# tdunnlab/scrubvae

Measured on AMD Instinct MI355X. Metric: pose-windows/sec (ELBO-match) on synthetic 64-frame mouse skeletons, higher is better.
Workload: dtype f32 (f16x3b3 split on the fp16 / bf16 matrix cores); 1 GPU; configs[2] full SC-VAE (conditional + grad_reversal x2 + adversarial_net), AdamW, batch 4096/GPU, window 64, 23 joints, z=32, channels [64,128,256,512,1024]; batch_per_gpu=4096, global_batch=4096, window=64, joints=23, launch=eager launches, inputs=resident in HBM, side_streams=2, parallelism=dp1, backend=none, ranks_seen=1, bn=single rank

## Files before the change

### scrubvae_amd/csrc/pose_tail.hip

```cpp
#include "svae_internal.h"
#include <cstdlib>

namespace svae {

struct TailArgs {
  const float* y;
  const float* offsets;
  const float* target;
  const float* root;
  const float* ext_dx6d;
  const float* ext_droot;
  float* x6d_hat;
  float* root_hat;
  float* loss_part;
  float* dy;
  float* pose_out;
  long long rows;
  int ld, J, ldt, ldo;
  int has_arena;
  int pre_tanh;
  float a0[3], a1[3];
  float jpe_scale, root_scale;
  svae_tree tree;
};

struct M3 {
  float m[9];
};

__device__ __forceinline__ M3 mul(const M3& a, const M3& b) {
  M3 c;
#pragma unroll
  for (int r = 0; r < 3; ++r)
#pragma unroll
    for (int k = 0; k < 3; ++k) c.m[r * 3 + k] = a.m[r * 3] * b.m[k] + a.m[r * 3 + 1] * b.m[3 + k] + a.m[r * 3 + 2] * b.m[6 + k];
  return c;
}
__device__ __forceinline__ M3 mul_tn(const M3& a, const M3& b) {
  M3 c;
#pragma unroll
  for (int r = 0; r < 3; ++r)
#pragma unroll
    for (int k = 0; k < 3; ++k) c.m[r * 3 + k] = a.m[r] * b.m[k] + a.m[3 + r] * b.m[3 + k] + a.m[6 + r] * b.m[6 + k];
  return c;
}
__device__ __forceinline__ M3 mul_nt(const M3& a, const M3& b) {
  M3 c;
#pragma unroll
  for (int r = 0; r < 3; ++r)
#pragma unroll
    for (int k = 0; k < 3; ++k)
      c.m[r * 3 + k] = a.m[r * 3] * b.m[k * 3] + a.m[r * 3 + 1] * b.m[k * 3 + 1] + a.m[r * 3 + 2] * b.m[k * 3 + 2];
  return c;
}

__device__ __forceinline__ void cross3(const float* a, const float* b, float* c) {
  c[0] = a[1] * b[2] - a[2] * b[1];
  c[1] = a[2] * b[0] - a[0] * b[2];
  c[2] = a[0] * b[1] - a[1] * b[0];
}

constexpr float K1_EPS = 1e-8f;

__device__ __forceinline__ M3 c6_to_mat(const float* a) {
  const float nx = sqrtf(a[0] * a[0] + a[1] * a[1] + a[2] * a[2]);
  const float ix = 1.f / (nx + K1_EPS);
  const float x[3] = {a[0] * ix, a[1] * ix, a[2] * ix};
  float zr[3];
  cross3(x, a + 3, zr);
  const float nz = sqrtf(zr[0] * zr[0] + zr[1] * zr[1] + zr[2] * zr[2]);
  const float iz = 1.f / (nz + K1_EPS);
  const float z[3] = {zr[0] * iz, zr[1] * iz, zr[2] * iz};
  float yv[3];
  cross3(z, x, yv);
  M3 M;
#pragma unroll
  for (int r = 0; r < 3; ++r) { M.m[r * 3] = x[r]; M.m[r * 3 + 1] = yv[r]; M.m[r * 3 + 2] = z[r]; }
  return M;
}

__device__ __forceinline__ void c6_to_mat_bwd(const float* a, const M3& dM, float* da) {
  const float nx = sqrtf(a[0] * a[0] + a[1] * a[1] + a[2] * a[2]);
  const float ix = 1.f / (nx + K1_EPS);
  const float x[3] = {a[0] * ix, a[1] * ix, a[2] * ix};
  float zr[3];
  cross3(x, a + 3, zr);
  const float nz = sqrtf(zr[0] * zr[0] + zr[1] * zr[1] + zr[2] * zr[2]);
  const float iz = 1.f / (nz + K1_EPS);
  const float z[3] = {zr[0] * iz, zr[1] * iz, zr[2] * iz};
  float gx[3] = {dM.m[0], dM.m[3], dM.m[6]}, gy[3] = {dM.m[1], dM.m[4], dM.m[7]}, gz[3] = {dM.m[2], dM.m[5], dM.m[8]};
  float t[3];
  cross3(x, gy, t);
  gz[0] += t[0]; gz[1] += t[1]; gz[2] += t[2];
  cross3(gy, z, t);
  gx[0] += t[0]; gx[1] += t[1]; gx[2] += t[2];
  const float dzr_dot = zr[0] * gz[0] + zr[1] * gz[1] + zr[2] * gz[2];
  const float kz = nz > 0.f ? dzr_dot * iz * iz / nz : 0.f;
  const float gzr[3] = {gz[0] * iz - zr[0] * kz, gz[1] * iz - zr[1] * kz, gz[2] * iz - zr[2] * kz};
  cross3(a + 3, gzr, t);
  gx[0] += t[0]; gx[1] += t[1]; gx[2] += t[2];
  cross3(gzr, x, da + 3);
  const float dx_dot = a[0] * gx[0] + a[1] * gx[1] + a[2] * gx[2];
  const float kx = nx > 0.f ? dx_dot * ix * ix / nx : 0.f;
  da[0] = gx[0] * ix - a[0] * kx;
  da[1] = gx[1] * ix - a[1] * kx;
  da[2] = gx[2] * ix - a[2] * kx;
}

template <int TR>
__global__ __launch_bounds__(64 * SVAE_MAX_CHAINS) void pose_tail_kernel(const TailArgs g) {
  extern __shared__ __attribute__((aligned(16))) float smem[];
  const int tid = threadIdx.x, nth = blockDim.x;
  const int wave = tid >> 6, lane = tid & 63;
  const int J = g.J, J3 = 3 * J, C6 = 6 * J;
  const int ldt = g.ldt, ldo = g.ldo;
  float* tile = smem;
  float* offs = tile + TR * ldt;
  float* pose = offs + TR * ldo;
  float* dm0 = pose + TR * ldo;
  float* red = dm0 + TR * 9;
  const long long r0 = (long long)blockIdx.x * TR;
  const int nrows = (int)((g.rows - r0) < TR ? (g.rows - r0) : TR);
  const int n_chains = g.tree.n_chains;

  {
    const int f4_per_row = g.ld / 4;
    const int total = nrows * f4_per_row;
    const float* src = g.y + r0 * g.ld;
    for (int e = tid; e < total; e += nth) {
      const int rr = e / f4_per_row, c = (e - rr * f4_per_row) * 4;
      const float4 v = *reinterpret_cast<const float4*>(src + (long long)e * 4);
      float* d = tile + rr * ldt + c;
      if (g.pre_tanh) { d[0] = tanhf(v.x); d[1] = tanhf(v.y); d[2] = tanhf(v.z); d[3] = tanhf(v.w); }
      else { d[0] = v.x; d[1] = v.y; d[2] = v.z; d[3] = v.w; }
    }
    const int tot3 = nrows * J3;
    const float* so = g.offsets + r0 * J3;
    for (int e = tid; e < tot3; e += nth) {
      const int rr = e / J3, c = e - rr * J3;
      offs[rr * ldo + c] = so[e];
    }
    for (int e = tid; e < TR * 9; e += nth) dm0[e] = 0.f;
  }
  __syncthreads();
  {
    const int tot6 = nrows * C6;
    float* dst = g.x6d_hat + r0 * C6;
    for (int e = tid; e < tot6; e += nth) {
      const int rr = e / C6, c = e - rr * C6;
      dst[e] = tile[rr * ldt + c];
    }
    if (g.has_arena) {
      float* dr = g.root_hat + r0 * 3;
      for (int e = tid; e < nrows * 3; e += nth) {
        const int rr = e / 3, k = e - rr * 3;
        dr[e] = 0.5f * (tile[rr * ldt + C6 + k] + 1.f) * (g.a1[k] - g.a0[k]) + g.a0[k];
      }
    }
  }

  const bool active = lane < nrows;
  const int lrow = lane < TR ? lane : 0;
  float* my = tile + lrow * ldt;
  float* myo = offs + lrow * ldo;
  float* myp = pose + lrow * ldo;
  const bool do_bwd = g.dy != nullptr;
  const bool chain_wave = wave < n_chains && g.tree.chain_len[wave < n_chains ? wave : 0] >= 2;
  const int ch = wave < n_chains ? wave : 0;
  const int len = g.tree.chain_len[ch];

  float a6[6];
  M3 M0;
  if (active) {
#pragma unroll
    for (int k = 0; k < 6; ++k) a6[k] = my[k];
    M0 = c6_to_mat(a6);
  }
  M3 Rc = M0;
  if (active && chain_wave) {
    M3& R = Rc;
    float acc[3] = {0.f, 0.f, 0.f};
    for (int i = 1; i < len; ++i) {
      const int j = g.tree.chain[ch][i];
#pragma unroll
      for (int k = 0; k < 6; ++k) a6[k] = my[6 * j + k];
      R = mul(R, c6_to_mat(a6));
      const float o0 = myo[3 * j], o1 = myo[3 * j + 1], o2 = myo[3 * j + 2];
#pragma unroll
      for (int r = 0; r < 3; ++r) {
        acc[r] += R.m[r * 3] * o0 + R.m[r * 3 + 1] * o1 + R.m[r * 3 + 2] * o2;
        myp[3 * j + r] = acc[r];
      }
    }
  }
  __syncthreads();

  float rl = 0.f;
  if (wave == 0 && active) {
    myp[0] = 0.f; myp[1] = 0.f; myp[2] = 0.f;
    for (int c = 0; c < n_chains; ++c) {
      const int cl = g.tree.chain_len[c];
      const int head = g.tree.chain[c][0];
      const float h0 = myp[3 * head], h1 = myp[3 * head + 1], h2 = myp[3 * head + 2];
      for (int i = 1; i < cl; ++i) {
        const int j = g.tree.chain[c][i];
        myp[3 * j] += h0; myp[3 * j + 1] += h1; myp[3 * j + 2] += h2;
      }
    }
  }
  const int root_wave = nth > 64 ? 1 : 0;
  if (wave == root_wave && active && g.has_arena) {
#pragma unroll
    for (int k = 0; k < 3; ++k) {
      const float xh = my[C6 + k];
      const float half = 0.5f * (g.a1[k] - g.a0[k]);
      const float rh = (xh + 1.f) * half + g.a0[k];
      const float d = rh - g.root[(r0 + lane) * 3 + k];
      rl += d * d;
      if (do_bwd) {
        float gk = 2.f * g.root_scale * d;
        if (g.ext_droot) gk += g.ext_droot[(r0 + lane) * 3 + k];
        my[C6 + k] = g.pre_tanh ? gk * half * (1.f - xh * xh) : gk * half;
      }
    }
  }
  if (wave == root_wave && active && do_bwd) {
    for (int c = C6 + (g.has_arena ? 3 : 0); c < g.ld; ++c) my[c] = 0.f;
  }
  __syncthreads();

  {
    float jpe = 0.f;
    const int tot3 = nrows * J3;
    const float* stg = g.target + r0 * J3;
    float* dp = g.pose_out ? g.pose_out + r0 * J3 : nullptr;
    for (int e = tid; e < tot3; e += nth) {
      const int rr = e / J3, c = e - rr * J3;
      const float pv = pose[rr * ldo + c];
      if (dp) dp[e] = pv;
      const float d = pv - stg[e];
      jpe += d * d;
      pose[rr * ldo + c] = 2.f * g.jpe_scale * d;
    }
    jpe = wave_sum(jpe);
    if (lane == 0) red[wave] = jpe;
  }
  __syncthreads();
  if (tid == 0) {
    float t = 0.f;
    for (int w = 0; w < nth / 64; ++w) t += red[w];
    g.loss_part[blockIdx.x * 2] = t;
  }
  if (do_bwd && wave == 0 && active) {
    for (int c = n_chains - 1; c >= 0; --c) {
      const int cl = g.tree.chain_len[c];
      for (int i = cl - 1; i >= 1; --i) {
        const int j = g.tree.chain[c][i], par = g.tree.chain[c][i - 1];
#pragma unroll
        for (int r = 0; r < 3; ++r) myp[3 * par + r] += myp[3 * j + r];
      }
    }
  }
  if (do_bwd) __syncthreads();

  M3 carry;
#pragma unroll
  for (int k = 0; k < 9; ++k) carry.m[k] = 0.f;
  if (do_bwd && active && chain_wave) {
    M3 P = Rc;
#pragma unroll
    for (int i = SVAE_MAX_CHAIN_LEN - 1; i >= 1; --i) {
      if (i < len) {
        const int j = g.tree.chain[ch][i];
        M3 D = carry;
#pragma unroll
        for (int r = 0; r < 3; ++r)
#pragma unroll
          for (int k = 0; k < 3; ++k) D.m[r * 3 + k] += myp[3 * j + r] * myo[3 * j + k];
#pragma unroll
        for (int k = 0; k < 6; ++k) a6[k] = my[6 * j + k];
        const M3 Mj = c6_to_mat(a6);
        {
          float inv[3];
#pragma unroll
          for (int c = 0; c < 3; ++c) inv[c] = 1.f / (Mj.m[c] * Mj.m[c] + Mj.m[3 + c] * Mj.m[3 + c] + Mj.m[6 + c] * Mj.m[6 + c]);
          M3 Q;
#pragma unroll
          for (int r = 0; r < 3; ++r)
#pragma unroll
            for (int k = 0; k < 3; ++k)
              Q.m[r * 3 + k] = P.m[r * 3] * inv[0] * Mj.m[k * 3] + P.m[r * 3 + 1] * inv[1] * Mj.m[k * 3 + 1] + P.m[r * 3 + 2] * inv[2] * Mj.m[k * 3 + 2];
          P = Q;
        }
        const M3 dMj = mul_tn(P, D);
        carry = mul_nt(D, Mj);
        float da[6];
        c6_to_mat_bwd(a6, dMj, da);
#pragma unroll
        for (int k = 0; k < 6; ++k) {
          float gk = da[k];
          if (g.ext_dx6d) gk += g.ext_dx6d[(r0 + lane) * C6 + 6 * j + k];
          my[6 * j + k] = g.pre_tanh ? gk * (1.f - a6[k] * a6[k]) : gk;
        }
      }
    }
  }
  if (do_bwd) {
    for (int c = 0; c < n_chains; ++c) {
      if (wave == c && chain_wave && active) {
        float* d = dm0 + lane * 9;
#pragma unroll
        for (int k = 0; k < 9; ++k) d[k] += carry.m[k];
      }
      __syncthreads();
    }
  }
  if (do_bwd && wave == 0 && active) {
    M3 dM0;
    const float* d = dm0 + lane * 9;
#pragma unroll
    for (int k = 0; k < 9; ++k) dM0.m[k] = d[k];
    float a0[6], da0[6];
#pragma unroll
    for (int k = 0; k < 6; ++k) a0[k] = my[k];
    c6_to_mat_bwd(a0, dM0, da0);
#pragma unroll
    for (int k = 0; k < 6; ++k) {
      float gk = da0[k];
      if (g.ext_dx6d) gk += g.ext_dx6d[(r0 + lane) * C6 + k];
      my[k] = g.pre_tanh ? gk * (1.f - a0[k] * a0[k]) : gk;
    }
  }
  if (wave == root_wave) {
    rl = wave_sum(rl);
    if (lane == 0) g.loss_part[blockIdx.x * 2 + 1] = rl;
  }
  __syncthreads();
  if (do_bwd) {
    const int f4_per_row = g.ld / 4;
    const int total = nrows * f4_per_row;
    float* dst = g.dy + r0 * g.ld;
    for (int e = tid; e < total; e += nth) {
      const int rr = e / f4_per_row, c = (e - rr * f4_per_row) * 4;
      const float* sp = tile + rr * ldt + c;
      *reinterpret_cast<float4*>(dst + (long long)e * 4) = make_float4(sp[0], sp[1], sp[2], sp[3]);
    }
  }
}

__device__ __forceinline__ void rot6d_rows(const float* d6, float* m ) {
  const float n1 = fmaxf(sqrtf(d6[0] * d6[0] + d6[1] * d6[1] + d6[2] * d6[2]), 1e-12f);
  const float b1[3] = {d6[0] / n1, d6[1] / n1, d6[2] / n1};
  const float dt = b1[0] * d6[3] + b1[1] * d6[4] + b1[2] * d6[5];
  const float u[3] = {d6[3] - dt * b1[0], d6[4] - dt * b1[1], d6[5] - dt * b1[2]};
  const float n2 = fmaxf(sqrtf(u[0] * u[0] + u[1] * u[1] + u[2] * u[2]), 1e-12f);
  const float b2[3] = {u[0] / n2, u[1] / n2, u[2] / n2};
  float b3[3];
  cross3(b1, b2, b3);
#pragma unroll
  for (int k = 0; k < 3; ++k) { m[k] = b1[k]; m[3 + k] = b2[k]; m[6 + k] = b3[k]; }
}

__device__ __forceinline__ void rot6d_rows_bwd(const float* d6, const float* g, float* dd) {
  const float n1r = sqrtf(d6[0] * d6[0] + d6[1] * d6[1] + d6[2] * d6[2]);
  const float n1 = fmaxf(n1r, 1e-12f);
  const float b1[3] = {d6[0] / n1, d6[1] / n1, d6[2] / n1};
  const float dt = b1[0] * d6[3] + b1[1] * d6[4] + b1[2] * d6[5];
  const float u[3] = {d6[3] - dt * b1[0], d6[4] - dt * b1[1], d6[5] - dt * b1[2]};
  const float n2r = sqrtf(u[0] * u[0] + u[1] * u[1] + u[2] * u[2]);
  const float n2 = fmaxf(n2r, 1e-12f);
  const float b2[3] = {u[0] / n2, u[1] / n2, u[2] / n2};
  float gb1[3] = {g[0], g[1], g[2]}, gb2[3] = {g[3], g[4], g[5]};
  const float gb3[3] = {g[6], g[7], g[8]};
  float t[3];
  cross3(b2, gb3, t);
  gb1[0] += t[0]; gb1[1] += t[1]; gb1[2] += t[2];
  cross3(gb3, b1, t);
  gb2[0] += t[0]; gb2[1] += t[1]; gb2[2] += t[2];
  float gu[3];
  if (n2r > 1e-12f) {
    const float d = b2[0] * gb2[0] + b2[1] * gb2[1] + b2[2] * gb2[2];
#pragma unroll
    for (int k = 0; k < 3; ++k) gu[k] = (gb2[k] - b2[k] * d) / n2;
  } else {
#pragma unroll
    for (int k = 0; k < 3; ++k) gu[k] = gb2[k] / n2;
  }
  const float gub1 = gu[0] * b1[0] + gu[1] * b1[1] + gu[2] * b1[2];
#pragma unroll
  for (int k = 0; k < 3; ++k) {
    dd[3 + k] = gu[k] - gub1 * b1[k];
    gb1[k] += -dt * gu[k] - gub1 * d6[3 + k];
  }
  if (n1r > 1e-12f) {
    const float d = b1[0] * gb1[0] + b1[1] * gb1[1] + b1[2] * gb1[2];
#pragma unroll
    for (int k = 0; k < 3; ++k) dd[k] = (gb1[k] - b1[k] * d) / n1;
  } else {
#pragma unroll
    for (int k = 0; k < 3; ++k) dd[k] = gb1[k] / n1;
  }
}

__global__ __launch_bounds__(256) void rot_loss_kernel(const float* __restrict__ x, const float* __restrict__ xh, float scale,
                                                        float* __restrict__ part, float* __restrict__ dxh, long long n) {
  __shared__ float red4[4];
  const long long i = (long long)blockIdx.x * 256 + threadIdx.x;
  float loss = 0.f;
  if (i < n) {
    float a[6], b[6], m1[9], m2[9];
#pragma unroll
    for (int k = 0; k < 6; ++k) { a[k] = x[i * 6 + k]; b[k] = xh[i * 6 + k]; }
    rot6d_rows(a, m1);
    rot6d_rows(b, m2);
    float ss = 0.f, d[9];
#pragma unroll
    for (int k = 0; k < 9; ++k) { d[k] = m2[k] - m1[k]; ss += d[k] * d[k]; }
    const float fro = sqrtf(ss);
    const float c = 0.35355339059327373f;
    float s = fro * c;
    const float lim = 1.f - 1e-7f;
    const bool clamped = s > lim;
    if (clamped) s = lim;
    loss = 2.f * asinf(s);
    if (dxh) {
      float gm[9];
      const float gs = (!clamped && fro > 0.f) ? scale * 2.f / sqrtf(1.f - s * s) * c / fro : 0.f;
#pragma unroll
      for (int k = 0; k < 9; ++k) gm[k] = gs * d[k];
      float dd[6];
      rot6d_rows_bwd(b, gm, dd);
#pragma unroll
      for (int k = 0; k < 6; ++k) dxh[i * 6 + k] = dd[k];
    }
  }
  const float t = block_sum_256(loss, red4);
  if (threadIdx.x == 0) part[blockIdx.x] = t;
}

}

using namespace svae;

static int tail_rows() {
  static int tr = 0;
  if (tr == 0) {
    const char* e = getenv("SVAE_TAIL_ROWS");
    const int v = e ? atoi(e) : 64;
    tr = (v == 64 || v == 48 || v == 32) ? v : 64;
  }
  return tr;
}

extern "C" int svae_tail_blocks(long long rows) { const int tr = tail_rows(); return (int)((rows + tr - 1) / tr); }

extern "C" int svae_pose_tail(const float* y, int ld, const float* offsets, const float* target_pose, const float* root,
                              const float* arena_host, const svae_tree* tree, float jpe_scale, float root_scale,
                              const float* ext_dx6d, const float* ext_droot, float* x6d_hat, float* root_hat, float* loss_part,
                              float* dy, float* pose_out, long long rows, int input_is_pre_tanh, void* stream) {
  SVAE_REQUIRE(y && offsets && target_pose && tree && x6d_hat && loss_part && rows > 0, SVAE_ERR_ARG, "pose_tail: null pointer");
  const int J = tree->n_joints;
  SVAE_REQUIRE(J >= 1 && J <= SVAE_MAX_JOINTS && tree->n_chains >= 0 && tree->n_chains <= SVAE_MAX_CHAINS, SVAE_ERR_SHAPE,
               "pose_tail: bad tree");
  SVAE_REQUIRE(ld % 4 == 0 && ld >= 6 * J + (arena_host ? 3 : 0) && aligned16(y) && (!dy || aligned16(dy)), SVAE_ERR_ALIGN,
               "pose_tail: ld %d too small or misaligned", ld);
  SVAE_REQUIRE(!arena_host || (root && root_hat), SVAE_ERR_ARG, "pose_tail: arena without root buffers");
  int seen[SVAE_MAX_JOINTS] = {0};
  seen[0] = 1;
  for (int c = 0; c < tree->n_chains; ++c) {
    const int len = tree->chain_len[c];
    SVAE_REQUIRE(len >= 1 && len <= SVAE_MAX_CHAIN_LEN, SVAE_ERR_SHAPE, "pose_tail: chain %d length %d", c, len);
    for (int i = 0; i < len; ++i) SVAE_REQUIRE(tree->chain[c][i] >= 0 && tree->chain[c][i] < J, SVAE_ERR_SHAPE, "pose_tail: joint id");
    SVAE_REQUIRE(seen[tree->chain[c][0]], SVAE_ERR_SHAPE, "pose_tail: chain %d starts at a joint not yet placed", c);
    for (int i = 1; i < len; ++i) {
      SVAE_REQUIRE(!seen[tree->chain[c][i]], SVAE_ERR_SHAPE, "pose_tail: joint %d placed twice", tree->chain[c][i]);
      seen[tree->chain[c][i]] = 1;
    }
  }
  for (int j = 0; j < J; ++j) SVAE_REQUIRE(seen[j], SVAE_ERR_SHAPE, "pose_tail: joint %d not covered by the kinematic tree", j);
  TailArgs g;
  memset(&g, 0, sizeof(g));
  g.y = y; g.offsets = offsets; g.target = target_pose; g.root = root; g.ext_dx6d = ext_dx6d; g.ext_droot = ext_droot;
  g.x6d_hat = x6d_hat; g.root_hat = root_hat; g.loss_part = loss_part; g.dy = dy; g.pose_out = pose_out;
  g.rows = rows; g.ld = ld; g.J = J;
  g.ldt = ld | 1;
  g.ldo = (3 * J) | 1;
  g.has_arena = arena_host != nullptr;
  g.pre_tanh = input_is_pre_tanh;
  if (arena_host)
    for (int k = 0; k < 3; ++k) { g.a0[k] = arena_host[k]; g.a1[k] = arena_host[3 + k]; }
  g.jpe_scale = jpe_scale; g.root_scale = root_scale;
  g.tree = *tree;
  const int n_waves = tree->n_chains >= 2 ? tree->n_chains : 2;
  const int tr = tail_rows();
  const size_t smem = (size_t)(tr * g.ldt + 2 * tr * g.ldo + tr * 9 + SVAE_MAX_CHAINS) * sizeof(float);
  SVAE_REQUIRE(smem <= 160 * 1024, SVAE_ERR_SHAPE, "pose_tail: LDS tile %zu B exceeds 160 KiB", smem);
  static DeviceOnce attr_set;
  int attr_dev;
  if (attr_set.need(&attr_dev)) {
    hipError_t e = hipFuncSetAttribute((const void*)pose_tail_kernel<64>, hipFuncAttributeMaxDynamicSharedMemorySize, 160 * 1024);
    if (e == hipSuccess) e = hipFuncSetAttribute((const void*)pose_tail_kernel<48>, hipFuncAttributeMaxDynamicSharedMemorySize, 160 * 1024);
    if (e == hipSuccess) e = hipFuncSetAttribute((const void*)pose_tail_kernel<32>, hipFuncAttributeMaxDynamicSharedMemorySize, 160 * 1024);
    SVAE_REQUIRE(e == hipSuccess, SVAE_ERR_LAUNCH, "pose_tail: hipFuncSetAttribute(MaxDynamicSharedMemorySize): %s", hipGetErrorString(e));
    attr_set.done(attr_dev);
  }
  const dim3 grid(svae_tail_blocks(rows)), block(64 * n_waves);
  if (tr == 64) hipLaunchKernelGGL(pose_tail_kernel<64>, grid, block, smem, (hipStream_t)stream, g);
  else if (tr == 48) hipLaunchKernelGGL(pose_tail_kernel<48>, grid, block, smem, (hipStream_t)stream, g);
  else hipLaunchKernelGGL(pose_tail_kernel<32>, grid, block, smem, (hipStream_t)stream, g);
  return check_launch("pose_tail");
}

extern "C" int svae_rot_blocks(long long n) { return (int)((n + 255) / 256); }

extern "C" int svae_rot_loss(const float* x6d, const float* x6d_hat, float scale, float* part, float* dx6d_hat, long long n,
                             void* stream) {
  SVAE_REQUIRE(x6d && x6d_hat && part && n > 0, SVAE_ERR_ARG, "rot_loss: bad args");
  hipLaunchKernelGGL(rot_loss_kernel, dim3(svae_rot_blocks(n)), dim3(256), 0, (hipStream_t)stream, x6d, x6d_hat, scale, part,
                     dx6d_hat, n);
  return check_launch("rot_loss");
}
```

Before: 292,000 windows/s.

## Restructure pose tail kernel to spread FK work across all threads per block

Rewrites the pose-tail forward-kinematics kernel so that a fixed 512-thread block parallelizes over (frame, joint) and (frame, chain) pairs instead of one lane per frame with one wave per chain. Per-joint 6D-to-rotation results and prefix rotations are cached in new LDS arrays. Root/head chain propagation and the gradient accumulation become precomputed head/mask tables instead of serial loops. Division by row widths is replaced with float reciprocal tricks, and the default tile rows drop from 64 to 32. This targets low occupancy and serial per-wave work, at the cost of more LDS, more barriers and float-based index division that could misround for large widths.

```diff
diff --git a/scrubvae_amd/csrc/pose_tail.hip b/scrubvae_amd/csrc/pose_tail.hip
--- a/scrubvae_amd/csrc/pose_tail.hip
+++ b/scrubvae_amd/csrc/pose_tail.hip
@@ -16,12 +16,15 @@
   float* dy;
   float* pose_out;
   long long rows;
-  int ld, J, ldt, ldo;
+  int ld, J, ldt, ldo, ldm, ldp;
   int has_arena;
   int pre_tanh;
   float a0[3], a1[3];
   float jpe_scale, root_scale;
+  float inv_f4, inv_j3, inv_c6, inv_pad;
   svae_tree tree;
+  int head[SVAE_MAX_JOINTS];
+  unsigned mask[SVAE_MAX_JOINTS];
 };
 
 struct M3 {
@@ -62,7 +65,7 @@
 
 constexpr float K1_EPS = 1e-8f;
 
-__device__ __forceinline__ M3 c6_to_mat(const float* a) {
+__device__ __forceinline__ void c6_to_xz(const float* a, float* xz) {
   const float nx = sqrtf(a[0] * a[0] + a[1] * a[1] + a[2] * a[2]);
   const float ix = 1.f / (nx + K1_EPS);
   const float x[3] = {a[0] * ix, a[1] * ix, a[2] * ix};
@@ -70,7 +73,12 @@
   cross3(x, a + 3, zr);
   const float nz = sqrtf(zr[0] * zr[0] + zr[1] * zr[1] + zr[2] * zr[2]);
   const float iz = 1.f / (nz + K1_EPS);
-  const float z[3] = {zr[0] * iz, zr[1] * iz, zr[2] * iz};
+#pragma unroll
+  for (int r = 0; r < 3; ++r) { xz[r] = x[r]; xz[3 + r] = zr[r] * iz; }
+}
+
+__device__ __forceinline__ M3 mat_from_xz(const float* xz) {
+  const float x[3] = {xz[0], xz[1], xz[2]}, z[3] = {xz[3], xz[4], xz[5]};
   float yv[3];
   cross3(z, x, yv);
   M3 M;
@@ -107,242 +115,346 @@
   da[2] = gx[2] * ix - a[2] * kx;
 }
 
+__device__ __forceinline__ int div_by(int e, float inv) { return (int)(((float)e + 0.5f) * inv); }
+
+constexpr int TAIL_THREADS = 512;
+constexpr int TAIL_WAVES = TAIL_THREADS / 64;
+
+struct RowWalk {
+  int rr, c, drr, dc, C;
+  __device__ __forceinline__ RowWalk(int tid, int C_, float inv) : C(C_) {
+    rr = div_by(tid, inv);
+    c = tid - rr * C;
+    drr = div_by(TAIL_THREADS, inv);
+    dc = TAIL_THREADS - drr * C;
+  }
+  __device__ __forceinline__ void next() {
+    rr += drr;
+    c += dc;
+    if (c >= C) { c -= C; ++rr; }
+  }
+};
+
+inline void tail_tables(TailArgs& g) {
+  const svae_tree& t = g.tree;
+  for (int j = 0; j < SVAE_MAX_JOINTS; ++j) { g.head[j] = 0; g.mask[j] = 1u << j; }
+  for (int c = t.n_chains - 1; c >= 0; --c)
+    for (int i = t.chain_len[c] - 1; i >= 1; --i) {
+      g.head[t.chain[c][i]] = t.chain[c][0];
+      g.mask[t.chain[c][i - 1]] |= g.mask[t.chain[c][i]];
+    }
+}
+
 template <int TR>
-__global__ __launch_bounds__(64 * SVAE_MAX_CHAINS) void pose_tail_kernel(const TailArgs g) {
+__global__ __launch_bounds__(TAIL_THREADS) void pose_tail_kernel(const TailArgs g) {
   extern __shared__ __attribute__((aligned(16))) float smem[];
-  const int tid = threadIdx.x, nth = blockDim.x;
+  constexpr int nth = TAIL_THREADS;
+  constexpr int NE = (TR * 3 * SVAE_MAX_JOINTS + nth - 1) / nth;
+  const int tid = threadIdx.x;
   const int wave = tid >> 6, lane = tid & 63;
   const int J = g.J, J3 = 3 * J, C6 = 6 * J;
-  const int ldt = g.ldt, ldo = g.ldo;
+  const int ldt = g.ldt, ldo = g.ldo, ldm = g.ldm, ldp = g.ldp;
   float* tile = smem;
   float* offs = tile + TR * ldt;
   float* pose = offs + TR * ldo;
-  float* dm0 = pose + TR * ldo;
-  float* red = dm0 + TR * 9;
+  float* mxz = pose + TR * ldo;
+  float* pre = mxz + TR * ldm;
+  float* red = pre + TR * ldp;
+  int* s_len = reinterpret_cast<int*>(red + 2 * TAIL_WAVES);
+  int* s_chain = s_len + SVAE_MAX_CHAINS;
+  int* s_head = s_chain + SVAE_MAX_CHAINS * SVAE_MAX_CHAIN_LEN;
+  int* s_mask = s_head + SVAE_MAX_JOINTS;
   const long long r0 = (long long)blockIdx.x * TR;
   const int nrows = (int)((g.rows - r0) < TR ? (g.rows - r0) : TR);
   const int n_chains = g.tree.n_chains;
+  const int tot3 = nrows * J3;
+  const bool do_bwd = g.dy != nullptr;
+
+  float tg[NE];
+  {
+    float of[NE];
+    const float* so = g.offsets + r0 * J3;
+    const float* stg = g.target + r0 * J3;
+#pragma unroll
+    for (int q = 0; q < NE; ++q) {
+      const int e = tid + q * nth;
+      of[q] = e < tot3 ? so[e] : 0.f;
+      tg[q] = e < tot3 ? stg[e] : 0.f;
+    }
+    const int f4_per_row = g.ld / 4;
+    const int total = nrows * f4_per_row;
+    const float* src = g.y + r0 * g.ld;
+    RowWalk w(tid, f4_per_row, g.inv_f4);
+    for (int e0 = tid; e0 < total; e0 += 4 * nth) {
+      float4 v[4];
+#pragma unroll
+      for (int u = 0; u < 4; ++u) {
+        const int e = e0 + u * nth;
+        v[u] = e < total ? *reinterpret_cast<const float4*>(src + (long long)e * 4) : make_float4(0.f, 0.f, 0.f, 0.f);
+      }
+#pragma unroll
+      for (int u = 0; u < 4; ++u, w.next()) {
+        if (e0 + u * nth < total) {
+          float* d = tile + w.rr * ldt + w.c * 4;
+          if (g.pre_tanh) { d[0] = tanhf(v[u].x); d[1] = tanhf(v[u].y); d[2] = tanhf(v[u].z); d[3] = tanhf(v[u].w); }
+          else { d[0] = v[u].x; d[1] = v[u].y; d[2] = v[u].z; d[3] = v[u].w; }
+        }
+      }
+    }
+    RowWalk w3(tid, J3, g.inv_j3);
+#pragma unroll
+    for (int q = 0; q < NE; ++q, w3.next())
+      if (tid + q * nth < tot3) offs[w3.rr * ldo + w3.c] = of[q];
+    for (int e = tid; e < SVAE_MAX_CHAINS * SVAE_MAX_CHAIN_LEN; e += nth) s_chain[e] = g.tree.chain[e / SVAE_MAX_CHAIN_LEN][e % SVAE_MAX_CHAIN_LEN];
+    for (int e = tid; e < SVAE_MAX_CHAINS; e += nth) s_len[e] = e < n_chains ? g.tree.chain_len[e] : 0;
+    for (int e = tid; e < SVAE_MAX_JOINTS; e += nth) { s_head[e] = g.head[e]; s_mask[e] = (int)g.mask[e]; }
+  }
+  __syncthreads();
+
+  {
+    const int tot6 = nrows * C6;
+    float* dst = g.x6d_hat + r0 * C6;
+    RowWalk w6(tid, C6, g.inv_c6);
+    for (int e = tid; e < tot6; e += nth, w6.next()) dst[e] = tile[w6.rr * ldt + w6.c];
+    float rl = 0.f;
+    if (g.has_arena) {
+      float* dr = g.root_hat + r0 * 3;
+      const float* sr = g.root + r0 * 3;
+      const float* se = g.ext_droot ? g.ext_droot + r0 * 3 : nullptr;
+      for (int e = tid; e < nrows * 3; e += nth) {
+        const int rr = e / 3, k = e - rr * 3;
+        float* t = tile + rr * ldt + C6 + k;
+        const float xh = *t;
+        dr[e] = 0.5f * (xh + 1.f) * (g.a1[k] - g.a0[k]) + g.a0[k];
+        const float half = 0.5f * (g.a1[k] - g.a0[k]);
+        const float d = (xh + 1.f) * half + g.a0[k] - sr[e];
+        rl += d * d;
+        if (do_bwd) {
+          float gk = 2.f * g.root_scale * d;
+          if (se) gk += se[e];
+          *t = g.pre_tanh ? gk * half * (1.f - xh * xh) : gk * half;
+        }
+      }
+    }
+    rl = wave_sum(rl);
+    if (lane == 0) red[TAIL_WAVES + wave] = rl;
+    const int c0 = C6 + (g.has_arena ? 3 : 0), npad = g.ld - c0;
+    if (do_bwd && npad > 0) {
+      for (int e = tid; e < nrows * npad; e += nth) {
+        const int rr = div_by(e, g.inv_pad);
+        tile[rr * ldt + c0 + (e - rr * npad)] = 0.f;
+      }
+    }
+    for (int e = tid; e < TR * J; e += nth) {
+      const int f = e % TR, j = e / TR;
+      if (f < nrows) {
+        float a6[6], xz[6];
+#pragma unroll
+        for (int k = 0; k < 6; ++k) a6[k] = tile[f * ldt + 6 * j + k];
+        c6_to_xz(a6, xz);
+#pragma unroll
+        for (int k = 0; k < 6; ++k) mxz[f * ldm + 6 * j + k] = xz[k];
+      }
+    }
+  }
+  __syncthreads();
+
+  for (int e = tid; e < TR * n_chains; e += nth) {
+    const int f = e % TR, c = e / TR, len = s_len[c];
+    if (f < nrows && len >= 2) {
+      int js[SVAE_MAX_CHAIN_LEN];
+#pragma unroll
+      for (int i = 0; i < SVAE_MAX_CHAIN_LEN; ++i) js[i] = s_chain[c * SVAE_MAX_CHAIN_LEN + i];
+      const float* fx = mxz + f * ldm;
+      const float* fo = offs + f * ldo;
+      float* fp = pose + f * ldo;
+      float* fq = pre + f * ldp;
+      M3 R = mat_from_xz(fx);
+      float acc[3] = {0.f, 0.f, 0.f};
+#pragma unroll
+      for (int i = 1; i < SVAE_MAX_CHAIN_LEN; ++i) {
+        if (i < len) {
+          const int j = js[i];
+          R = mul(R, mat_from_xz(fx + 6 * j));
+#pragma unroll
+          for (int k = 0; k < 9; ++k) fq[9 * j + k] = R.m[k];
+          const float o0 = fo[3 * j], o1 = fo[3 * j + 1], o2 = fo[3 * j + 2];
+#pragma unroll
+          for (int r = 0; r < 3; ++r) {
+            acc[r] += R.m[r * 3] * o0 + R.m[r * 3 + 1] * o1 + R.m[r * 3 + 2] * o2;
+            fp[3 * j + r] = acc[r];
+          }
+        }
+      }
+    }
+  }
+  __syncthreads();
+
+  float pv[NE];
+  {
+    RowWalk w3(tid, J3, g.inv_j3);
+#pragma unroll
+    for (int q = 0; q < NE; ++q, w3.next()) {
+      if (tid + q * nth < tot3) {
+        const int j = w3.c / 3, r = w3.c - 3 * j;
+        const float* p = pose + w3.rr * ldo;
+        float v = 0.f;
+        if (j != 0) {
+          v = p[w3.c];
+          int h = s_head[j];
+          for (int n = 0; h != 0 && n < SVAE_MAX_CHAINS; ++n) { v += p[3 * h + r]; h = s_head[h]; }
+        }
+        pv[q] = v;
+      }
+    }
+  }
+  __syncthreads();
+
+  {
+    float jpe = 0.f;
+    float* dp = g.pose_out ? g.pose_out + r0 * J3 : nullptr;
+    RowWalk w3(tid, J3, g.inv_j3);
+#pragma unroll
+    for (int q = 0; q < NE; ++q, w3.next()) {
+      const int e = tid + q * nth;
+      if (e < tot3) {
+        if (dp) dp[e] = pv[q];
+        const float d = pv[q] - tg[q];
+        jpe += d * d;
+        pose[w3.rr * ldo + w3.c] = 2.f * g.jpe_scale * d;
+      }
+    }
+    jpe = wave_sum(jpe);
+    if (lane == 0) red[wave] = jpe;
+  }
+  __syncthreads();
+  if (tid == 0) {
+    float t = 0.f, u = 0.f;
+    for (int w = 0; w < TAIL_WAVES; ++w) { t += red[w]; u += red[TAIL_WAVES + w]; }
+    g.loss_part[blockIdx.x * 2] = t;
+    g.loss_part[blockIdx.x * 2 + 1] = u;
+  }
+  if (!do_bwd) return;
+
+  {
+    float gs[NE];
+#pragma unroll
+    for (int q = 0; q < NE; ++q) {
+      const int e = tid + q * nth, f = e % TR, c = e / TR;
+      gs[q] = 0.f;
+      if (c >= 3 && c < J3 && f < nrows) {
+        const int j = c / 3, r = c - 3 * j;
+        const float* p = pose + f * ldo + r;
+        float s = 0.f;
+        for (unsigned m = (unsigned)s_mask[j]; m != 0; m &= m - 1) s += p[3 * (__ffs(m) - 1)];
+        gs[q] = s;
+      }
+    }
+    __syncthreads();
+#pragma unroll
+    for (int q = 0; q < NE; ++q) {
+      const int e = tid + q * nth, f = e % TR, c = e / TR;
+      if (c >= 3 && c < J3 && f < nrows) pose[f * ldo + c] = gs[q];
+    }
+  }
+  __syncthreads();
+
+  for (int e = tid; e < TR * n_chains; e += nth) {
+    const int f = e % TR, c = e / TR, len = s_len[c];
+    if (f < nrows && len >= 2) {
+      int js[SVAE_MAX_CHAIN_LEN];
+#pragma unroll
+      for (int i = 0; i < SVAE_MAX_CHAIN_LEN; ++i) js[i] = s_chain[c * SVAE_MAX_CHAIN_LEN + i];
+      float* fx = mxz + f * ldm;
+      const float* fo = offs + f * ldo;
+      float* fp = pose + f * ldo;
+      float* fq = pre + f * ldp;
+      M3 carry;
+#pragma unroll
+      for (int k = 0; k < 9; ++k) carry.m[k] = 0.f;
+#pragma unroll
+      for (int i = SVAE_MAX_CHAIN_LEN - 1; i >= 1; --i) {
+        if (i < len) {
+          const int j = js[i];
+          M3 D = carry;
+#pragma unroll
+          for (int r = 0; r < 3; ++r)
+#pragma unroll
+            for (int k = 0; k < 3; ++k) D.m[r * 3 + k] += fp[3 * j + r] * fo[3 * j + k];
+          M3 P;
+          if (i >= 2) {
+#pragma unroll
+            for (int k = 0; k < 9; ++k) P.m[k] = fq[9 * js[i - 1] + k];
+          } else {
+            P = mat_from_xz(fx);
+          }
+          const M3 Mj = mat_from_xz(fx + 6 * j);
+          const M3 dMj = mul_tn(P, D);
+          carry = mul_nt(D, Mj);
+#pragma unroll
+          for (int k = 0; k < 9; ++k) fq[9 * j + k] = dMj.m[k];
+          if (i == 1) {
+#pragma unroll
+            for (int k = 0; k < 6; ++k) fx[6 * j + k] = carry.m[k];
+#pragma unroll
+            for (int k = 0; k < 3; ++k) fp[3 * j + k] = carry.m[6 + k];
+          }
+        }
+      }
+    }
+  }
+  __syncthreads();
+
+  for (int e = tid; e < TR * 9; e += nth) {
+    const int f = e % TR, k = e / TR;
+    if (f < nrows) {
+      float s = 0.f;
+      for (int c = 0; c < n_chains; ++c) {
+        if (s_len[c] >= 2) {
+          const int j1 = s_chain[c * SVAE_MAX_CHAIN_LEN + 1];
+          s += k < 6 ? mxz[f * ldm + 6 * j1 + k] : pose[f * ldo + 3 * j1 + k - 6];
+        }
+      }
+      pre[f * ldp + k] = s;
+    }
+  }
+  __syncthreads();
+
+  if (g.ext_dx6d) {
+    const int tot6 = nrows * C6;
+    const float* se = g.ext_dx6d + r0 * C6;
+    RowWalk w6(tid, C6, g.inv_c6);
+    for (int e = tid; e < tot6; e += nth, w6.next()) mxz[w6.rr * ldm + w6.c] = se[e];
+    __syncthreads();
+  }
+
+  for (int e = tid; e < TR * J; e += nth) {
+    const int f = e % TR, j = e / TR;
+    if (f < nrows) {
+      float a6[6], da[6];
+      M3 dM;
+#pragma unroll
+      for (int k = 0; k < 6; ++k) a6[k] = tile[f * ldt + 6 * j + k];
+#pragma unroll
+      for (int k = 0; k < 9; ++k) dM.m[k] = pre[f * ldp + 9 * j + k];
+      c6_to_mat_bwd(a6, dM, da);
+#pragma unroll
+      for (int k = 0; k < 6; ++k) {
+        float gk = da[k];
+        if (g.ext_dx6d) gk += mxz[f * ldm + 6 * j + k];
+        tile[f * ldt + 6 * j + k] = g.pre_tanh ? gk * (1.f - a6[k] * a6[k]) : gk;
+      }
+    }
+  }
+  __syncthreads();
 
   {
     const int f4_per_row = g.ld / 4;
     const int total = nrows * f4_per_row;
-    const float* src = g.y + r0 * g.ld;
-    for (int e = tid; e < total; e += nth) {
-      const int rr = e / f4_per_row, c = (e - rr * f4_per_row) * 4;
-      const float4 v = *reinterpret_cast<const float4*>(src + (long long)e * 4);
-      float* d = tile + rr * ldt + c;
-      if (g.pre_tanh) { d[0] = tanhf(v.x); d[1] = tanhf(v.y); d[2] = tanhf(v.z); d[3] = tanhf(v.w); }
-      else { d[0] = v.x; d[1] = v.y; d[2] = v.z; d[3] = v.w; }
-    }
-    const int tot3 = nrows * J3;
-    const float* so = g.offsets + r0 * J3;
-    for (int e = tid; e < tot3; e += nth) {
-      const int rr = e / J3, c = e - rr * J3;
-      offs[rr * ldo + c] = so[e];
-    }
-    for (int e = tid; e < TR * 9; e += nth) dm0[e] = 0.f;
-  }
-  __syncthreads();
-  {
-    const int tot6 = nrows * C6;
-    float* dst = g.x6d_hat + r0 * C6;
-    for (int e = tid; e < tot6; e += nth) {
-      const int rr = e / C6, c = e - rr * C6;
-      dst[e] = tile[rr * ldt + c];
-    }
-    if (g.has_arena) {
-      float* dr = g.root_hat + r0 * 3;
-      for (int e = tid; e < nrows * 3; e += nth) {
-        const int rr = e / 3, k = e - rr * 3;
-        dr[e] = 0.5f * (tile[rr * ldt + C6 + k] + 1.f) * (g.a1[k] - g.a0[k]) + g.a0[k];
-      }
-    }
-  }
-
-  const bool active = lane < nrows;
-  const int lrow = lane < TR ? lane : 0;
-  float* my = tile + lrow * ldt;
-  float* myo = offs + lrow * ldo;
-  float* myp = pose + lrow * ldo;
-  const bool do_bwd = g.dy != nullptr;
-  const bool chain_wave = wave < n_chains && g.tree.chain_len[wave < n_chains ? wave : 0] >= 2;
-  const int ch = wave < n_chains ? wave : 0;
-  const int len = g.tree.chain_len[ch];
-
-  float a6[6];
-  M3 M0;
-  if (active) {
-#pragma unroll
-    for (int k = 0; k < 6; ++k) a6[k] = my[k];
-    M0 = c6_to_mat(a6);
-  }
-  M3 Rc = M0;
-  if (active && chain_wave) {
-    M3& R = Rc;
-    float acc[3] = {0.f, 0.f, 0.f};
-    for (int i = 1; i < len; ++i) {
-      const int j = g.tree.chain[ch][i];
-#pragma unroll
-      for (int k = 0; k < 6; ++k) a6[k] = my[6 * j + k];
-      R = mul(R, c6_to_mat(a6));
-      const float o0 = myo[3 * j], o1 = myo[3 * j + 1], o2 = myo[3 * j + 2];
-#pragma unroll
-      for (int r = 0; r < 3; ++r) {
-        acc[r] += R.m[r * 3] * o0 + R.m[r * 3 + 1] * o1 + R.m[r * 3 + 2] * o2;
-        myp[3 * j + r] = acc[r];
-      }
-    }
-  }
-  __syncthreads();
-
-  float rl = 0.f;
-  if (wave == 0 && active) {
-    myp[0] = 0.f; myp[1] = 0.f; myp[2] = 0.f;
-    for (int c = 0; c < n_chains; ++c) {
-      const int cl = g.tree.chain_len[c];
-      const int head = g.tree.chain[c][0];
-      const float h0 = myp[3 * head], h1 = myp[3 * head + 1], h2 = myp[3 * head + 2];
-      for (int i = 1; i < cl; ++i) {
-        const int j = g.tree.chain[c][i];
-        myp[3 * j] += h0; myp[3 * j + 1] += h1; myp[3 * j + 2] += h2;
-      }
-    }
-  }
-  const int root_wave = nth > 64 ? 1 : 0;
-  if (wave == root_wave && active && g.has_arena) {
-#pragma unroll
-    for (int k = 0; k < 3; ++k) {
-      const float xh = my[C6 + k];
-      const float half = 0.5f * (g.a1[k] - g.a0[k]);
-      const float rh = (xh + 1.f) * half + g.a0[k];
-      const float d = rh - g.root[(r0 + lane) * 3 + k];
-      rl += d * d;
-      if (do_bwd) {
-        float gk = 2.f * g.root_scale * d;
-        if (g.ext_droot) gk += g.ext_droot[(r0 + lane) * 3 + k];
-        my[C6 + k] = g.pre_tanh ? gk * half * (1.f - xh * xh) : gk * half;
-      }
-    }
-  }
-  if (wave == root_wave && active && do_bwd) {
-    for (int c = C6 + (g.has_arena ? 3 : 0); c < g.ld; ++c) my[c] = 0.f;
-  }
-  __syncthreads();
-
-  {
-    float jpe = 0.f;
-    const int tot3 = nrows * J3;
-    const float* stg = g.target + r0 * J3;
-    float* dp = g.pose_out ? g.pose_out + r0 * J3 : nullptr;
-    for (int e = tid; e < tot3; e += nth) {
-      const int rr = e / J3, c = e - rr * J3;
-      const float pv = pose[rr * ldo + c];
-      if (dp) dp[e] = pv;
-      const float d = pv - stg[e];
-      jpe += d * d;
-      pose[rr * ldo + c] = 2.f * g.jpe_scale * d;
-    }
-    jpe = wave_sum(jpe);
-    if (lane == 0) red[wave] = jpe;
-  }
-  __syncthreads();
-  if (tid == 0) {
-    float t = 0.f;
-    for (int w = 0; w < nth / 64; ++w) t += red[w];
-    g.loss_part[blockIdx.x * 2] = t;
-  }
-  if (do_bwd && wave == 0 && active) {
-    for (int c = n_chains - 1; c >= 0; --c) {
-      const int cl = g.tree.chain_len[c];
-      for (int i = cl - 1; i >= 1; --i) {
-        const int j = g.tree.chain[c][i], par = g.tree.chain[c][i - 1];
-#pragma unroll
-        for (int r = 0; r < 3; ++r) myp[3 * par + r] += myp[3 * j + r];
-      }
-    }
-  }
-  if (do_bwd) __syncthreads();
-
-  M3 carry;
-#pragma unroll
-  for (int k = 0; k < 9; ++k) carry.m[k] = 0.f;
-  if (do_bwd && active && chain_wave) {
-    M3 P = Rc;
-#pragma unroll
-    for (int i = SVAE_MAX_CHAIN_LEN - 1; i >= 1; --i) {
-      if (i < len) {
-        const int j = g.tree.chain[ch][i];
-        M3 D = carry;
-#pragma unroll
-        for (int r = 0; r < 3; ++r)
-#pragma unroll
-          for (int k = 0; k < 3; ++k) D.m[r * 3 + k] += myp[3 * j + r] * myo[3 * j + k];
-#pragma unroll
-        for (int k = 0; k < 6; ++k) a6[k] = my[6 * j + k];
-        const M3 Mj = c6_to_mat(a6);
-        {
-          float inv[3];
-#pragma unroll
-          for (int c = 0; c < 3; ++c) inv[c] = 1.f / (Mj.m[c] * Mj.m[c] + Mj.m[3 + c] * Mj.m[3 + c] + Mj.m[6 + c] * Mj.m[6 + c]);
-          M3 Q;
-#pragma unroll
-          for (int r = 0; r < 3; ++r)
-#pragma unroll
-            for (int k = 0; k < 3; ++k)
-              Q.m[r * 3 + k] = P.m[r * 3] * inv[0] * Mj.m[k * 3] + P.m[r * 3 + 1] * inv[1] * Mj.m[k * 3 + 1] + P.m[r * 3 + 2] * inv[2] * Mj.m[k * 3 + 2];
-          P = Q;
-        }
-        const M3 dMj = mul_tn(P, D);
-        carry = mul_nt(D, Mj);
-        float da[6];
-        c6_to_mat_bwd(a6, dMj, da);
-#pragma unroll
-        for (int k = 0; k < 6; ++k) {
-          float gk = da[k];
-          if (g.ext_dx6d) gk += g.ext_dx6d[(r0 + lane) * C6 + 6 * j + k];
-          my[6 * j + k] = g.pre_tanh ? gk * (1.f - a6[k] * a6[k]) : gk;
-        }
-      }
-    }
-  }
-  if (do_bwd) {
-    for (int c = 0; c < n_chains; ++c) {
-      if (wave == c && chain_wave && active) {
-        float* d = dm0 + lane * 9;
-#pragma unroll
-        for (int k = 0; k < 9; ++k) d[k] += carry.m[k];
-      }
-      __syncthreads();
-    }
-  }
-  if (do_bwd && wave == 0 && active) {
-    M3 dM0;
-    const float* d = dm0 + lane * 9;
-#pragma unroll
-    for (int k = 0; k < 9; ++k) dM0.m[k] = d[k];
-    float a0[6], da0[6];
-#pragma unroll
-    for (int k = 0; k < 6; ++k) a0[k] = my[k];
-    c6_to_mat_bwd(a0, dM0, da0);
-#pragma unroll
-    for (int k = 0; k < 6; ++k) {
-      float gk = da0[k];
-      if (g.ext_dx6d) gk += g.ext_dx6d[(r0 + lane) * C6 + k];
-      my[k] = g.pre_tanh ? gk * (1.f - a0[k] * a0[k]) : gk;
-    }
-  }
-  if (wave == root_wave) {
-    rl = wave_sum(rl);
-    if (lane == 0) g.loss_part[blockIdx.x * 2 + 1] = rl;
-  }
-  __syncthreads();
-  if (do_bwd) {
-    const int f4_per_row = g.ld / 4;
-    const int total = nrows * f4_per_row;
     float* dst = g.dy + r0 * g.ld;
-    for (int e = tid; e < total; e += nth) {
-      const int rr = e / f4_per_row, c = (e - rr * f4_per_row) * 4;
-      const float* sp = tile + rr * ldt + c;
+    RowWalk w(tid, f4_per_row, g.inv_f4);
+    for (int e = tid; e < total; e += nth, w.next()) {
+      const float* sp = tile + w.rr * ldt + w.c * 4;
       *reinterpret_cast<float4*>(dst + (long long)e * 4) = make_float4(sp[0], sp[1], sp[2], sp[3]);
     }
   }
@@ -446,8 +558,8 @@
   static int tr = 0;
   if (tr == 0) {
     const char* e = getenv("SVAE_TAIL_ROWS");
-    const int v = e ? atoi(e) : 64;
-    tr = (v == 64 || v == 48 || v == 32) ? v : 64;
+    const int v = e ? atoi(e) : 32;
+    tr = (v == 64 || v == 32 || v == 16) ? v : 32;
   }
   return tr;
 }
@@ -485,29 +597,33 @@
   g.rows = rows; g.ld = ld; g.J = J;
   g.ldt = ld | 1;
   g.ldo = (3 * J) | 1;
+  g.ldm = (6 * J) | 1;
+  g.ldp = (9 * J) | 1;
   g.has_arena = arena_host != nullptr;
   g.pre_tanh = input_is_pre_tanh;
   if (arena_host)
     for (int k = 0; k < 3; ++k) { g.a0[k] = arena_host[k]; g.a1[k] = arena_host[3 + k]; }
   g.jpe_scale = jpe_scale; g.root_scale = root_scale;
+  g.inv_f4 = 1.f / (float)(ld / 4); g.inv_j3 = 1.f / (float)(3 * J); g.inv_c6 = 1.f / (float)(6 * J);
+  g.inv_pad = 1.f / (float)(ld - 6 * J - (arena_host ? 3 : 0) > 0 ? ld - 6 * J - (arena_host ? 3 : 0) : 1);
   g.tree = *tree;
-  const int n_waves = tree->n_chains >= 2 ? tree->n_chains : 2;
+  tail_tables(g);
   const int tr = tail_rows();
-  const size_t smem = (size_t)(tr * g.ldt + 2 * tr * g.ldo + tr * 9 + SVAE_MAX_CHAINS) * sizeof(float);
+  const size_t smem = (size_t)(tr * (g.ldt + 2 * g.ldo + g.ldm + g.ldp) + 2 * TAIL_WAVES + SVAE_MAX_CHAINS * (1 + SVAE_MAX_CHAIN_LEN) + 2 * SVAE_MAX_JOINTS) * sizeof(float);
   SVAE_REQUIRE(smem <= 160 * 1024, SVAE_ERR_SHAPE, "pose_tail: LDS tile %zu B exceeds 160 KiB", smem);
   static DeviceOnce attr_set;
   int attr_dev;
   if (attr_set.need(&attr_dev)) {
     hipError_t e = hipFuncSetAttribute((const void*)pose_tail_kernel<64>, hipFuncAttributeMaxDynamicSharedMemorySize, 160 * 1024);
-    if (e == hipSuccess) e = hipFuncSetAttribute((const void*)pose_tail_kernel<48>, hipFuncAttributeMaxDynamicSharedMemorySize, 160 * 1024);
     if (e == hipSuccess) e = hipFuncSetAttribute((const void*)pose_tail_kernel<32>, hipFuncAttributeMaxDynamicSharedMemorySize, 160 * 1024);
+    if (e == hipSuccess) e = hipFuncSetAttribute((const void*)pose_tail_kernel<16>, hipFuncAttributeMaxDynamicSharedMemorySize, 160 * 1024);
     SVAE_REQUIRE(e == hipSuccess, SVAE_ERR_LAUNCH, "pose_tail: hipFuncSetAttribute(MaxDynamicSharedMemorySize): %s", hipGetErrorString(e));
     attr_set.done(attr_dev);
   }
-  const dim3 grid(svae_tail_blocks(rows)), block(64 * n_waves);
+  const dim3 grid(svae_tail_blocks(rows)), block(TAIL_THREADS);
   if (tr == 64) hipLaunchKernelGGL(pose_tail_kernel<64>, grid, block, smem, (hipStream_t)stream, g);
-  else if (tr == 48) hipLaunchKernelGGL(pose_tail_kernel<48>, grid, block, smem, (hipStream_t)stream, g);
-  else hipLaunchKernelGGL(pose_tail_kernel<32>, grid, block, smem, (hipStream_t)stream, g);
+  else if (tr == 32) hipLaunchKernelGGL(pose_tail_kernel<32>, grid, block, smem, (hipStream_t)stream, g);
+  else hipLaunchKernelGGL(pose_tail_kernel<16>, grid, block, smem, (hipStream_t)stream, g);
   return check_launch("pose_tail");
 }
 
```

Result: no change. 293,300 windows/s (median of 6 runs) (+0.5%).
